# shirokumakur0/Riemannian-interior-point-trust-region-method

Measured on AMD Instinct MI355X. Metric: outer RIPTRM iterations/sec, batched NonnegPCA n=4000, 1/2/4/8 MI355X, higher is better.
Workload: dtype f64

## Files before the change

riemannian-interior-point-trust-region-method_amd/csrc/riptrm_device.h:

```cpp
#pragma once
#include <stdint.h>
#include "../../include/riptrm.h"

namespace riptrm {

constexpr int TS = 128;
constexpr int SP_WAVES = 8;
constexpr int SP_THREADS = SP_WAVES * 64;
constexpr int GV_THREADS = 256;
constexpr int GV_RW = 4;
constexpr int GV_RB = (GV_THREADS / 64) * GV_RW;
constexpr int ST_THREADS = 512;
constexpr int ST_WAVES = ST_THREADS / 64;

enum Vec : int {
  V_X = 0, V_Y, V_ETA, V_HETA,
  V_SX, V_X0, V_Y0, V_SX0, V_XPREV, V_R, V_IN0, V_IN1, V_OUT0, V_OUT1, V_YNEW, V_C,
  V_XI, V_YI, V_SXI,
  NVEC
};

enum St : int {
  ST_PHASE = 0, ST_MODE, ST_OUTER_IT, ST_INNER_IT, ST_MU_IDX, ST_MU, ST_DELTA, ST_DELTA0,
  ST_DELTA_STEP, ST_T_START, ST_T_INNER, ST_TOLL, ST_TOLC,
  ST_XX, ST_XSX, ST_YX, ST_COEF, ST_FCUR,
  ST_EPE, ST_EPD, ST_DPD, ST_ZR, ST_NORMR0, ST_MODEL, ST_J, ST_TCG_STOP,
  ST_NORMDX, ST_XDX, ST_MINX, ST_MINY, ST_COMPL, ST_XFEAS, ST_YFEAS,
  ST_HASMIN, ST_MINEIG, ST_MINEIG_OK,
  ST_HOT_END,
  ST_TCG_TOTAL = 40, ST_INNER_TOTAL, ST_PASSES, ST_LOG_COUNT, ST_LOG_OVERFLOW, ST_STOP_CODE,
  ST_STOP_RUNTIME, ST_RESIDUAL,
  ST_I_HAS, ST_I_NUM, ST_I_STATUS, ST_I_TR, ST_I_DXTYPE, ST_I_NORMDX, ST_I_MINX, ST_I_MINY,
  ST_I_COMPL, ST_I_HASRATIO, ST_I_RATIO, ST_I_RU, ST_I_DC, ST_I_HASMIN, ST_I_MINEIG,
  ST_ERROR, ST_LOG_BASE, ST_RHS,
  ST_N_USED
};
constexpr int ST_N = 72;
constexpr int ST_HOT = ST_HOT_END;
static_assert(ST_HOT_END <= 40, "hot scalar slots overflow into cold ones");
static_assert(ST_N_USED <= ST_N, "state slots overflow");

enum Phase : int {
  PH_IDLE = 0, PH_START, PH_AFTER_SX0, PH_TCG, PH_TRIAL, PH_PAUSED, PH_DONE,
  PH_TCGO_START, PH_TCGO_SX, PH_ERROR,
  PH_TRS, PH_TRS_END,
  PH_TRS_HOST, PH_MINEIG_HOST, PH_MINEIG_END
};

enum Mode : int { MODE_SOLVE = 0, MODE_TCG_ONLY = 1 };

struct Layout {
  int32_t n, batch, cap, layout, nt;
  int32_t reps;
  int64_t ld;
  int64_t off_vec, off_state, off_stats, off_log, off_pbuf, off_lists, off_req, off_cnt;
  int64_t off_rvec, off_rstate, off_rstats, off_rreq, off_pbuf2, off_sync, sync_bytes, off_tgrid, tgrid_bytes;
  int64_t total;
};

inline int64_t round_up(int64_t a, int64_t m) { return (a + m - 1) / m * m; }

__host__ __device__ inline int64_t log_slot(int64_t k, int64_t cap) {
  if (k < cap) return k;
  const int64_t h = cap / 2, t = cap - h;
  return h + (k - h) % t;
}
inline int64_t ld_of(int32_t n) { return round_up(n > 0 ? n : 1, TS); }
inline int64_t rows_of(int32_t n) { return round_up(n > 0 ? n : 1, 32); }
inline int32_t nt_of(int32_t n) { return (int32_t)(ld_of(n) / TS); }
inline int64_t ntiles_of(int32_t n) { const int64_t t = nt_of(n); return t * (t + 1) / 2; }
constexpr int SB = 2;
constexpr int SW = SB * TS;
inline int32_t nst_of(int32_t n) { return (nt_of(n) + SB - 1) / SB; }
inline int64_t nsup_of(int32_t n) { const int64_t t = nst_of(n); return t * (t + 1) / 2; }
inline int64_t pgrid_of(int32_t n) {
  const int64_t a = (int64_t)nt_of(n) * nt_of(n) * TS, b = (int64_t)nst_of(n) * nst_of(n) * SW;
  return a > b ? a : b;
}
#ifndef RIPTRM_MM_KZ
#define RIPTRM_MM_KZ 4
#endif
constexpr int MM_KZ = RIPTRM_MM_KZ;

inline int32_t edge_w_of(int32_t n) {
  return (int32_t)round_up((int64_t)(n > 0 ? n : 1) - (int64_t)(nt_of(n) - 1) * TS, 32);
}
__host__ __device__ inline int64_t sym_off(int I, int J, int nt, int wl) {
  const int64_t F = (int64_t)TS * TS;
  return F * ((int64_t)I * (nt - 1) - (int64_t)I * (I - 1) / 2) + (int64_t)I * TS * wl + (int64_t)(J - I) * F;
}

inline int64_t s_elems_of(int32_t n, int32_t layout) {
  if (layout == RIPTRM_LAYOUT_SYMTILE) {
    const int nt = nt_of(n), wl = edge_w_of(n);
    return sym_off(nt - 1, nt - 1, nt, wl) + (int64_t)wl * wl;
  }
  return rows_of(n) * ld_of(n);
}

constexpr int PERSIST_MAX_WG = 256;
constexpr int PERSIST_MAX_N = 2048;
inline int32_t persist_reps_of(int32_t n, int32_t batch, int32_t layout) {
  if (layout != RIPTRM_LAYOUT_SYMTILE || n > PERSIST_MAX_N) return 0;
  const int64_t t = ntiles_of(n);
  return (int64_t)batch * t <= PERSIST_MAX_WG ? (int32_t)t : 0;
}

inline Layout make_layout(int32_t n, int32_t batch, int32_t cap, int32_t layout) {
  Layout L;
  L.n = n; L.batch = batch; L.cap = cap; L.ld = ld_of(n); L.layout = layout; L.nt = nt_of(n);
  int64_t o = 0;
  L.off_vec = o;   o += (int64_t)NVEC * batch * L.ld * 8;               o = round_up(o, 256);
  L.off_state = o; o += (int64_t)batch * ST_N * 8;                       o = round_up(o, 256);
  L.off_stats = o; o += (int64_t)batch * RIPTRM_STAT_NFIELDS * 8;        o = round_up(o, 256);
  L.off_log = o;   o += (int64_t)batch * cap * RIPTRM_LOG_NFIELDS * 8;   o = round_up(o, 256);
  L.off_pbuf = o;
  if (layout == RIPTRM_LAYOUT_SYMTILE) o += (int64_t)2 * batch * pgrid_of(n) * 8;
  if (layout == RIPTRM_LAYOUT_SHARED) o += (int64_t)MM_KZ * 2 * batch * L.ld * 8;
  o = round_up(o, 256);
  L.off_lists = o; o += (int64_t)4 * batch * 4;                          o = round_up(o, 256);
  L.off_req = o;   o += (int64_t)batch * 4;                              o = round_up(o, 256);
  L.off_cnt = o;   o += 64;
  L.reps = persist_reps_of(n, batch, layout);
  const int64_t bs = L.reps > 0 ? (int64_t)batch * (L.reps - 1) : 0;
  L.off_rvec = o;   o += (int64_t)NVEC * bs * L.ld * 8;                  o = round_up(o, 256);
  L.off_rstate = o; o += bs * ST_N * 8;                                  o = round_up(o, 256);
  L.off_rstats = o; o += bs * RIPTRM_STAT_NFIELDS * 8;                   o = round_up(o, 256);
  L.off_rreq = o;   o += bs * 4;                                         o = round_up(o, 256);
  L.off_pbuf2 = o;  if (L.reps > 0) o += (int64_t)2 * batch * pgrid_of(n) * 8;  o = round_up(o, 256);
  L.off_sync = o;
  L.sync_bytes = L.reps > 0 ? round_up((int64_t)batch * 4, 16) + (int64_t)2 * batch * 8 + 16 : 0;
  o += L.sync_bytes;                                                     o = round_up(o, 256);
  L.off_tgrid = o;
  L.tgrid_bytes = L.reps > 0 ? (int64_t)2 * batch * nt_of(n) * nt_of(n) * TS * 16 : 0;
  o += L.tgrid_bytes;                                                    o = round_up(o, 256);
  L.total = o;
  return L;
}

struct DevParams {
  const double* S;
  int64_t inst_stride;
  int64_t ld;
  int32_t n, batch, cap;
  int32_t nrb;
  int32_t layout;
  int32_t nt;
  int32_t ntiles;
  int32_t wl;
  int32_t nst, nsup;
  int32_t smode;
  int32_t sup_dyn;
  double* pbuf;
  int32_t pbatch;
  double* vec;
  double* st;
  double* stats;
  double* log;
  int32_t* lists;
  int32_t* req;
  int32_t* cnt;
  const double* mu_tab;
  const double* tolL_tab;
  const double* tolC_tab;
  int32_t tab_len;
  int32_t outer_target;
  double clock_hz;
  int32_t trs_hbm;
  riptrm_options opt;
};

}
```

riemannian-interior-point-trust-region-method_amd/csrc/riptrm_kernels.hip:

```cpp
#include <hip/hip_runtime.h>
#include <math.h>
#include <string>
#include <vector>
#include <cstring>
#include <cstdio>
#include <type_traits>
#include "riptrm_device.h"
#include "riptrm_ctx.h"
#include "riptrm_wave.h"
#include "riptrm_trs.h"

namespace riptrm {

#pragma clang fp contract(off)

typedef double dbl2 __attribute__((ext_vector_type(2)));

__device__ __forceinline__ double* vp(const DevParams& P, int k, int b) {
  return P.vec + ((int64_t)k * P.batch + b) * P.ld;
}

__device__ __forceinline__ int32_t le_make(int b, int nrhs) { return b * 2 + (nrhs - 1); }
__device__ __forceinline__ int le_b(int32_t e) { return e >> 1; }
__device__ __forceinline__ int le_nrhs(int32_t e) { return (e & 1) + 1; }
// ... 173 lines not shown
  const int lane = (int)__lane_id();
#pragma unroll
  for (int k = 0; k < 4; ++k) {
    swap32(a[k], a[k + 4]);
    a[k] = a[k] + a[k + 4];
  }
#pragma unroll
  for (int k = 0; k < 2; ++k) {
    swap16(a[k], a[k + 2]);
    a[k] = a[k] + a[k + 2];
  }
  const double r0 = a[0], r1 = a[1];
  const bool b3 = (lane & 8) != 0;
  const double snd = b3 ? r0 : r1, kp = b3 ? r1 : r0;
  double v = kp + xor_lane(snd, 8);
  v += xor_lane(v, 4);
  v += xor_lane(v, 2);
  v += xor_lane(v, 1);
  return v;
}

template <int NR>
__device__ __forceinline__ void spass_tile(const DevParams& P, int b, int t) {
  int I, J;
  tile_ij(t, P.nt, I, J);
  const int lane = (int)__lane_id();
  const int w = __builtin_amdgcn_readfirstlane(threadIdx.x >> 6);
  const int nt = P.nt, wl = P.wl;
  const int rowsT = (I == nt - 1) ? wl : TS;
  const int colsT = (J == nt - 1) ? wl : TS;
  const bool cl = 2 * lane < colsT;
  const double* __restrict__ T = P.S + (int64_t)b * P.inst_stride + sym_off(I, J, nt, wl);
  const double* __restrict__ v0 = vp(P, V_IN0, b);
  const double* __restrict__ v1 = vp(P, V_IN1, b);
  const dbl2 vj0 = *(const dbl2*)(v0 + J * TS + 2 * lane);
  dbl2 vj1 = dbl2{0.0, 0.0};
  if (NR == 2) vj1 = *(const dbl2*)(v1 + J * TS + 2 * lane);
  const int64_t nn = (int64_t)P.nt * P.nt * TS;
  double* __restrict__ pb0 = P.pbuf + (int64_t)b * nn;
  double* __restrict__ pb1 = P.pbuf + ((int64_t)P.pbatch + b) * nn;
  double c0x = 0.0, c0y = 0.0, c1x = 0.0, c1y = 0.0;
  const int rrow = 4 * ((lane >> 5) & 1) + 2 * ((lane >> 4) & 1) + ((lane >> 3) & 1);
  constexpr int ROWS = TS / SP_WAVES;
#pragma unroll 1
  for (int rb = 0; rb < ROWS / 8; ++rb) {
    const int r0 = w * ROWS + rb * 8;
    if (r0 >= rowsT) break;
    dbl2 sv[8];
#pragma unroll
    for (int k = 0; k < 8; ++k)
      sv[k] = cl ? __builtin_nontemporal_load((const dbl2*)(T + (r0 + k) * colsT + 2 * lane)) : dbl2{0.0, 0.0};
    double a[8];
#pragma unroll
    for (int k = 0; k < 8; ++k) {
      const double vi0 = v0[I * TS + r0 + k];
      a[k] = __builtin_fma(sv[k].y, vj0.y, sv[k].x * vj0.x);
      c0x = __builtin_fma(sv[k].x, vi0, c0x);
      c0y = __builtin_fma(sv[k].y, vi0, c0y);
    }
    const double s0 = reduce_scatter8(a);
    if ((lane & 7) == 0) pb0[((int64_t)I * P.nt + J) * TS + r0 + rrow] = s0;
    if (NR == 2) {
#pragma unroll
      for (int k = 0; k < 8; ++k) {
        const double vi1 = v1[I * TS + r0 + k];
        a[k] = __builtin_fma(sv[k].y, vj1.y, sv[k].x * vj1.x);
        c1x = __builtin_fma(sv[k].x, vi1, c1x);
        c1y = __builtin_fma(sv[k].y, vi1, c1y);
      }
      const double s1 = reduce_scatter8(a);
      if ((lane & 7) == 0) pb1[((int64_t)I * P.nt + J) * TS + r0 + rrow] = s1;
    }
  }
  if (I != J) {
    __shared__ double cs[2][SP_WAVES][TS];
    cs[0][w][2 * lane] = c0x;
    cs[0][w][2 * lane + 1] = c0y;
    if (NR == 2) {
      cs[1][w][2 * lane] = c1x;
      cs[1][w][2 * lane + 1] = c1y;
    }
    __syncthreads();
    if (threadIdx.x < TS) {
      const int c = threadIdx.x;
      double s0 = cs[0][0][c];
#pragma unroll
      for (int q = 1; q < SP_WAVES; ++q) s0 += cs[0][q][c];
      pb0[((int64_t)J * P.nt + I) * TS + c] = s0;
      if (NR == 2) {
        double s1 = cs[1][0][c];
#pragma unroll
        for (int q = 1; q < SP_WAVES; ++q) s1 += cs[1][q][c];
        pb1[((int64_t)J * P.nt + I) * TS + c] = s1;
      }
    }
  }
}

__global__ void __launch_bounds__(SP_THREADS, 4) k_spass_sym(DevParams P, int list_in, int zero_cnt) {
  if (zero_cnt >= 0 && blockIdx.x == 0 && threadIdx.x == 0) P.cnt[zero_cnt] = 0;
  const int slot = blockIdx.x / P.ntiles;
  const int nact = P.cnt[list_in];
  const int32_t e = P.lists[list_in * P.batch + slot];
  if (slot >= nact) return;
  const int b = le_b(e);
  const int t = blockIdx.x - slot * P.ntiles;
  if (le_nrhs(e) == 2) spass_tile<2>(P, b, t);
  else spass_tile<1>(P, b, t);
}

constexpr int SUP_OCAP = 15360;
constexpr int SUP_MAXU = SUP_OCAP / (2 * SW);

typedef double (*sup_red_t)[SP_WAVES][SW];

template <int NR>
__device__ __forceinline__ void sup_unit(const DevParams& P, int b, int Pq, int Qq, sup_red_t red, double* out, int rsel) {
  const int lane = (int)__lane_id();
  const int w = __builtin_amdgcn_readfirstlane(threadIdx.x >> 6);
  const int nt = P.nt, wl = P.wl;
  constexpr int ROWS = TS / SP_WAVES;
  const double* __restrict__ Sb = P.S + (int64_t)b * P.inst_stride;
  const double* __restrict__ v0 = vp(P, V_IN0, b);
  const double* __restrict__ v1 = vp(P, V_IN1, b);
  const int rrow = 4 * ((lane >> 5) & 1) + 2 * ((lane >> 4) & 1) + ((lane >> 3) & 1);
  double racc[NR][SB][2];
#pragma unroll
  for (int k = 0; k < NR; ++k)
#pragma unroll
    for (int i = 0; i < SB; ++i) racc[k][i][0] = racc[k][i][1] = 0.0;
  if (NR == 2) __syncthreads();
  const int r0sel = NR == 2 ? 0 : rsel;
#pragma unroll
  for (int k = 0; k < NR; ++k)
    for (int jl = 0; jl < SB; ++jl) {
      red[r0sel + k][w][jl * TS + 2 * lane] = 0.0;
      red[r0sel + k][w][jl * TS + 2 * lane + 1] = 0.0;
    }
#pragma unroll
  for (int il = 0; il < SB; ++il) {
    const int I = SB * Pq + il;
    if (I >= nt) break;
    const int rowsT = (I == nt - 1) ? wl : TS;
    constexpr bool hoist = NR == 1;
    double vih[ROWS];
    if (hoist) {
#pragma unroll
      for (int k = 0; k < ROWS; ++k) vih[k] = v0[I * TS + w * ROWS + k];
    }
#pragma unroll 1
    for (int jl = 0; jl < SB; ++jl) {
      const int J = SB * Qq + jl;
      if (J >= nt || J < I) continue;
      const int colsT = (J == nt - 1) ? wl : TS;
      const bool cl = 2 * lane < colsT;
      const double* __restrict__ T = Sb + sym_off(I, J, nt, wl);
      const dbl2 vj0 = *(const dbl2*)(v0 + J * TS + 2 * lane);
      dbl2 vj1 = dbl2{0.0, 0.0};
      if (NR == 2) vj1 = *(const dbl2*)(v1 + J * TS + 2 * lane);
      double vi0[ROWS], vi1[ROWS];
#pragma unroll
      for (int k = 0; k < ROWS; ++k) {
        vi0[k] = hoist ? vih[k] : v0[I * TS + w * ROWS + k];
        vi1[k] = NR == 2 ? v1[I * TS + w * ROWS + k] : 0.0;
      }
      __builtin_amdgcn_sched_barrier(0);
      double c0x = 0.0, c0y = 0.0, c1x = 0.0, c1y = 0.0;
      dbl2 sv2[ROWS / 8][8];
#pragma unroll
      for (int rb = 0; rb < ROWS / 8; ++rb)
#pragma unroll
        for (int k = 0; k < 8; ++k) {
          const int row = w * ROWS + rb * 8 + k;
          const bool ok = cl && row < rowsT;
          const dbl2 x = __builtin_nontemporal_load((const dbl2*)(T + (row < rowsT ? row : 0) * colsT + (cl ? 2 * lane : 0)));
          sv2[rb][k] = ok ? x : dbl2{0.0, 0.0};
        }
#pragma unroll
      for (int rb = 0; rb < ROWS / 8; ++rb) {
        const int r0 = w * ROWS + rb * 8;
        if (r0 >= rowsT) break;
        const dbl2 (&sv)[8] = sv2[rb];
        double a[8];
#pragma unroll
        for (int k = 0; k < 8; ++k) {
          const double vi = vi0[rb * 8 + k];
          a[k] = __builtin_fma(sv[k].y, vj0.y, sv[k].x * vj0.x);
          c0x = __builtin_fma(sv[k].x, vi, c0x);
          c0y = __builtin_fma(sv[k].y, vi, c0y);
        }
        racc[0][il][rb] += reduce_scatter8(a);
        if (NR == 2) {
#pragma unroll
          for (int k = 0; k < 8; ++k) {
            const double vi = vi1[rb * 8 + k];
            a[k] = __builtin_fma(sv[k].y, vj1.y, sv[k].x * vj1.x);
            c1x = __builtin_fma(sv[k].x, vi, c1x);
            c1y = __builtin_fma(sv[k].y, vi, c1y);
          }
          racc[NR - 1][il][rb] += reduce_scatter8(a);
        }
      }
      if (I != J) {
        red[r0sel][w][jl * TS + 2 * lane] += c0x;
        red[r0sel][w][jl * TS + 2 * lane + 1] += c0y;
        if (NR == 2) {
          red[NR - 1][w][jl * TS + 2 * lane] += c1x;
          red[NR - 1][w][jl * TS + 2 * lane + 1] += c1y;
        }
      }
    }
  }
  if ((lane & 7) == 0) {
#pragma unroll
    for (int k = 0; k < NR; ++k)
#pragma unroll
      for (int il = 0; il < SB; ++il) {
        out[(2 * k) * SW + il * TS + w * ROWS + rrow] = racc[k][il][0];
        out[(2 * k) * SW + il * TS + w * ROWS + 8 + rrow] = racc[k][il][1];
      }
  }
  __syncthreads();
  for (int t = threadIdx.x; t < NR * SW; t += SP_THREADS) {
    const int k = t / SW, c = t - k * SW;
    double cs = red[r0sel + k][0][c];
#pragma unroll
    for (int q = 1; q < SP_WAVES; ++q) cs += red[r0sel + k][q][c];
    if (Pq == Qq) out[(2 * k) * SW + c] += cs;
    else out[(2 * k + 1) * SW + c] = cs;
  }
  if (NR == 2) __syncthreads();
}

__device__ __forceinline__ void sup_flush(const DevParams& P, const double* outb, const int (*meta)[2], int nslot,
                                          int list_in) {
  __syncthreads();
  const int64_t nn = (int64_t)P.nst * P.nst * SW;
  int off = 0;
  for (int s = 0; s < nslot; ++s) {
    const int u = meta[s][0], nr = meta[s][1];
    const int slot = u / P.nsup;
    const int b = le_b(P.lists[list_in * P.batch + slot]);
    int Pq, Qq;
    tile_ij(u - slot * P.nsup, P.nst, Pq, Qq);
    const int t = threadIdx.x, side = t / SW, c = t - side * SW;
    for (int k = 0; k < nr; ++k) {
      double* pb = P.pbuf + ((int64_t)k * P.pbatch + b) * nn;
      if (side == 0) pb[((int64_t)Pq * P.nst + Qq) * SW + c] = outb[off + (2 * k) * SW + c];
      else if (Pq != Qq) pb[((int64_t)Qq * P.nst + Pq) * SW + c] = outb[off + (2 * k + 1) * SW + c];
    }
    off += nr * 2 * SW;
  }
  __syncthreads();
}

__global__ void __launch_bounds__(SP_THREADS, 1) k_spass_sup(DevParams P, int list_in, int zero_cnt) {
  static_assert(SP_THREADS == 2 * SW, "sup_flush: one thread per element of the two sides");
  __shared__ double red[2][SP_WAVES][SW];
  __shared__ double outb[SUP_OCAP];
  __shared__ int meta[SUP_MAXU][2];
  __shared__ int tick_next;
  if (zero_cnt >= 0 && blockIdx.x == 0 && threadIdx.x == 0) P.cnt[zero_cnt] = 0;
  const int nact = P.cnt[list_in];
  const int total = nact * P.nsup;
  int used = 0, nslot = 0, rsel = 0;
  const bool dyn = P.sup_dyn != 0;
  unsigned int* tick = (unsigned int*)P.cnt + 8 + list_in;
  unsigned int* done = (unsigned int*)P.cnt + 12 + list_in;
  int u = blockIdx.x;
  if (dyn) {
    if (threadIdx.x == 0) tick_next = (int)atomicAdd(tick, 1u);
    __syncthreads();
    u = tick_next;
  }
  while (u < total) {
    unsigned int pre = 0;
    if (dyn && threadIdx.x == 0) pre = atomicAdd(tick, 1u);
    const int slot = u / P.nsup;
    const int32_t e = P.lists[list_in * P.batch + slot];
    const int b = le_b(e), nr = le_nrhs(e);
    int Pq, Qq;
    tile_ij(u - slot * P.nsup, P.nst, Pq, Qq);
    if (used + nr * 2 * SW > SUP_OCAP) {
      sup_flush(P, outb, meta, nslot, list_in);
      used = 0;
      nslot = 0;
    }
    if (nr == 2) {
      sup_unit<2>(P, b, Pq, Qq, red, outb + used, 0);
    } else {
      sup_unit<1>(P, b, Pq, Qq, red, outb + used, rsel);
      rsel ^= 1;
    }
    if (threadIdx.x == 0) {
      meta[nslot][0] = u;
      meta[nslot][1] = nr;
    }
    used += nr * 2 * SW;
    ++nslot;
    if (dyn) {
      __syncthreads();
      if (threadIdx.x == 0) tick_next = (int)pre;
      __syncthreads();
      u = tick_next;
    } else {
      u += gridDim.x;
    }
  }
  if (nslot > 0) sup_flush(P, outb, meta, nslot, list_in);
  if (dyn && threadIdx.x == 0) {
    if (atomicAdd(done, 1u) == gridDim.x - 1) {
      atomicExch(tick, 0u);
      atomicExch(done, 0u);
    }
  }
}

typedef double dbl4 __attribute__((ext_vector_type(4)));
typedef __attribute__((address_space(3))) unsigned char lds_u8;
#ifndef RIPTRM_MM_WAVES
#define RIPTRM_MM_WAVES 16
#endif
constexpr int MM_WAVES = RIPTRM_MM_WAVES;
typedef __attribute__((address_space(3))) dbl2 lds_dbl2;
#ifndef RIPTRM_MM_NST
#define RIPTRM_MM_NST 3
#endif

template <int N>
__device__ __forceinline__ void mm_wait_barrier() {
#define MM_WB_CASE(K) else if constexpr (N == K) asm volatile("s_waitcnt vmcnt(" #K ")\n\ts_barrier" ::: "memory");
  if constexpr (N == 0) asm volatile("s_waitcnt vmcnt(0)\n\ts_barrier" ::: "memory");
  MM_WB_CASE(1) MM_WB_CASE(2) MM_WB_CASE(3) MM_WB_CASE(4) MM_WB_CASE(5) MM_WB_CASE(6) MM_WB_CASE(7)
  MM_WB_CASE(8) MM_WB_CASE(9) MM_WB_CASE(10) MM_WB_CASE(11) MM_WB_CASE(12)
#undef MM_WB_CASE
  else static_assert(N < 0, "mm_wait_barrier: add the count");
}

template <int WM, int RT>
struct MmShape {
  static constexpr int NW = MM_WAVES;
  static constexpr int CT = 16 * WM;
  static constexpr int NWR = NW < RT / 16 ? NW : RT / 16;
  static constexpr int NWC = NW / NWR < WM ? NW / NWR : WM, NACT = NWR * NWC;
  static constexpr int WMW = WM / NWC;
  static constexpr int RW = RT / NWR, WN = RW / 16;
  static constexpr int VT = CT * 256;
  static constexpr int STAGE = VT + RT * 256;
  static constexpr int VW = NW < CT / 4 ? NW : CT / 4, VP = CT / 4 / VW;
  static constexpr int SW = NW < RT / 4 ? NW : RT / 4, SP = RT / 4 / SW;
  static constexpr int NST = RIPTRM_MM_NST >= 3 && 3 * STAGE + 32 * 4 <= 160 * 1024 ? 3 : 2;
  static_assert(WMW >= 1 && WN >= 1 && WM % NWC == 0 && VP * VW * 4 == CT && SP * SW * 4 == RT, "tile shape");
};

template <int WM, int RT, typename SlotOf>
__device__ __forceinline__ void mm_tile(const DevParams& P, lds_u8* smem, const int32_t* lst, int vk, int which, int nv,
                                        SlotOf slot_of, int z, int i0, int rows) {
  using Sh = MmShape<WM, RT>;
  constexpr int CT = Sh::CT, WN = Sh::WN, WMW = Sh::WMW, RW = Sh::RW, NWR = Sh::NWR;
  constexpr int VT = Sh::VT, STAGE = Sh::STAGE, VP = Sh::VP, SP = Sh::SP, NST = Sh::NST;
  constexpr int VW = Sh::VW, SW = Sh::SW, NACT = Sh::NACT;
  const int lane = threadIdx.x & 63, w = __builtin_amdgcn_readfirstlane((int)threadIdx.x >> 6);
  const int wr = w % NWR, wc = w / NWR;
  const int r = lane & 15, q = lane >> 4;
  const int64_t ld = P.ld;
  const double* vsrc[VP];
  const double* ssrc[SP];
#pragma unroll
  for (int p = 0; p < VP; ++p) {
    const int row = 4 * (VP * w + p) + q;
    vsrc[p] = vp(P, vk, le_b(lst[slot_of(min(row, nv - 1))])) + 2 * (r ^ (row & 15));
  }
#pragma unroll
  for (int p = 0; p < SP; ++p) {
    const int row = 4 * (SP * w + p) + q;
    const int i = min(i0 + row, rows - 1);
    ssrc[p] = P.S + (int64_t)i * ld + 2 * (r ^ (row & 15));
  }
  const int nch = (int)(ld / 32), per = (nch + MM_KZ - 1) / MM_KZ;
  const int lo = z * per, hi = min(nch, lo + per);
  auto issue = [&](int ch, int buf) {
    const int64_t k0 = (int64_t)ch * 32;
    lds_u8* vb = smem + buf * STAGE;
#pragma unroll
    for (int p = 0; p < VP; ++p)
      if (VW == Sh::NW || w < VW)
        __builtin_amdgcn_global_load_lds((const void*)(vsrc[p] + k0), vb + 4 * (VP * w + p) * 256, 16, 0, 0);
#pragma unroll
    for (int p = 0; p < SP; ++p)
      if (SW == Sh::NW || w < SW)
        __builtin_amdgcn_global_load_lds((const void*)(ssrc[p] + k0), vb + VT + 4 * (SP * w + p) * 256, 16, 0, 0);
  };
  dbl4 acc[WMW][WN];
#pragma unroll
  for (int a = 0; a < WMW; ++a)
#pragma unroll
    for (int c = 0; c < WN; ++c) acc[a][c] = dbl4{0.0, 0.0, 0.0, 0.0};
  const bool live = w < NACT && i0 + RW * wr < P.n && 16 * WMW * wc < nv;
  if (lo < hi) issue(lo, 0);
  if (NST == 3 && lo + 1 < hi) issue(lo + 1, 1);
  int s = 0;
  for (int ch = lo; ch < hi; ++ch) {
    if (NST == 3 && ch + 1 < hi) {
      if (w < VW && w < SW) mm_wait_barrier<VP + SP>();
      else if (w < VW) mm_wait_barrier<VP>();
      else if (w < SW) mm_wait_barrier<SP>();
      else mm_wait_barrier<0>();
    } else {
      mm_wait_barrier<0>();
    }
    if (ch + NST - 1 < hi) issue(ch + NST - 1, s == 0 ? NST - 1 : s - 1);
    const int sc = s;
    s = s + 1 == NST ? 0 : s + 1;
    if (!live) continue;
    const lds_u8* vb = smem + sc * STAGE + 16 * WMW * wc * 256;
    const lds_u8* sb = smem + sc * STAGE + VT + RW * wr * 256;
    dbl2 fa[2][WMW], fb[2][WN];
    auto frag = [&](int jj, int u) {
      const int off = ((4 * q + jj) ^ r) * 16;
#pragma unroll
      for (int a = 0; a < WMW; ++a) fa[u][a] = *(const lds_dbl2*)(vb + (16 * a + r) * 256 + off);
#pragma unroll
      for (int c = 0; c < WN; ++c) fb[u][c] = *(const lds_dbl2*)(sb + (16 * c + r) * 256 + off);
    };
    frag(0, 0);
#pragma unroll
    for (int jj = 0; jj < 4; ++jj) {
      const int u = jj & 1;
      if (jj < 3) frag(jj + 1, u ^ 1);
#pragma unroll
      for (int mm = 0; mm < 2; ++mm)
#pragma unroll
        for (int a = 0; a < WMW; ++a)
#pragma unroll
          for (int c = 0; c < WN; ++c)
            acc[a][c] = __builtin_amdgcn_mfma_f64_16x16x4f64(mm ? fa[u][a].y : fa[u][a].x, mm ? fb[u][c].y : fb[u][c].x,
                                                             acc[a][c], 0, 0, 0);
    }
  }
  (void)CT;
  if (!live) return;
  double* slab = P.pbuf + ((int64_t)z * 2 + which) * P.batch * ld;
#pragma unroll
  for (int a = 0; a < WMW; ++a)
#pragma unroll
    for (int g = 0; g < 4; ++g) {
      const int v = 16 * (WMW * wc + a) + q + 4 * g;
      if (v >= nv) continue;
      double* o = slab + (int64_t)le_b(lst[slot_of(v)]) * ld;
#pragma unroll
      for (int c = 0; c < WN; ++c) {
        const int i = i0 + RW * wr + 16 * c + r;
        if (i < P.n) o[i] = acc[a][c][g];
      }
    }
}

template <int WM0, int RT>
constexpr int mm_shm() { return MmShape<WM0, RT>::NST * MmShape<WM0, RT>::STAGE + 32 * 4; }
// ... 2202 lines not shown
                     c->L.reps - 1);
  HIPCHK(c, hipGetLastError());
  return RIPTRM_OK;
}

static void reset_groups(riptrm_ctx* c) {
  c->parity[0] = c->parity[1] = 0;
  c->active_bound[0] = c->active_bound[1] = 0;
}

static int kick(riptrm_ctx* c);
static int run_steps(riptrm_ctx* c, int steps, int* n_active);

extern "C++" template <int K>
static hipError_t persist_launch(riptrm_ctx* c, unsigned grid, DevParams p, RepBlock rq, PersistSync sy, int steps) {
  const size_t shm = (size_t)TS * TS * sizeof(double);
  if (c->persist_req == 2) {
    hipLaunchKernelGGL(k_persist<K>, dim3(grid), dim3(ST_THREADS), shm, c->stream, p, rq, sy, steps);
    return hipGetLastError();
  }
  if (c->persist_req == 3 && !c->persist_launched) return hipErrorCooperativeLaunchTooLarge;
  void* args[] = {&p, &rq, &sy, &steps};
  return hipLaunchCooperativeKernel((const void*)k_persist<K>, dim3(grid), dim3(ST_THREADS), args, (unsigned)shm,
                                    c->stream);
}

static int persist_run(riptrm_ctx* c, int steps, int* n_active) {
  const PersistSync sy = persist_sync(c);
  HIPCHK(c, hipMemsetAsync(c->ws + c->L.off_sync, 0, (size_t)(c->L.off_tgrid - c->L.off_sync + c->L.tgrid_bytes),
                           c->stream));
  if (steps > 0) {
    int i0 = -1, i1 = -1;
    hipEvent_t e0 = nullptr, e1 = nullptr;
    if (c->prof && (e0 = prof_event(c, &i0)) && (e1 = prof_event(c, &i1))) HIPCHK(c, hipEventRecord(e0, c->stream));
    const unsigned grid = (unsigned)(c->P.batch * c->L.reps);
    const DevParams Q = persist_params(c);
    const RepBlock rq{Q.vec, Q.st, Q.stats, Q.req, Q.batch};
    static_assert(PERSIST_MAX_N <= 4 * ST_THREADS, "k_persist<4> covers every persistent shape");
    const hipError_t le = c->P.n <= 2 * ST_THREADS ? persist_launch<2>(c, grid, params_for(c, 0), rq, sy, steps)
                                                    : persist_launch<4>(c, grid, params_for(c, 0), rq, sy, steps);
    if (le != hipSuccess) {
      (void)hipGetLastError();
      if (c->persist_launched)
        return fail(c, RIPTRM_E_HIP, std::string("persistent lock-step launch refused mid-solve: ") + hipGetErrorString(le));
      c->persist_on = false;
      c->persist_fallbacks++;
      c->ev_used -= (e0 ? 1 : 0) + (e1 ? 1 : 0);
      reset_groups(c);
      HIPCHK(c, hipMemsetAsync(c->P.cnt, 0, 4 * sizeof(int32_t), c->stream));
      if (int rc = kick(c)) return rc;
      return run_steps(c, steps, n_active);
    }
    c->persist_launched = true;
    if (c->prof && e1) {
      HIPCHK(c, hipEventRecord(e1, c->stream));
      c->ev_state.push_back({i0, i1});
    }
  }
  hipLaunchKernelGGL(k_persist_count, dim3(1), dim3(256), 0, c->stream, c->P, c->parity[0]);
  HIPCHK(c, hipGetLastError());
  int32_t h = 0;
  uint32_t flag = 0;
  HIPCHK(c, hipMemcpyAsync(&h, c->P.cnt + c->parity[0], sizeof(int32_t), hipMemcpyDeviceToHost, c->stream));
  HIPCHK(c, hipMemcpyAsync(&flag, sy.flag, sizeof(uint32_t), hipMemcpyDeviceToHost, c->stream));
  HIPCHK(c, hipStreamSynchronize(c->stream));
  if (c->prof) prof_collect(c);
  c->active_bound[0] = h;
  if (n_active) *n_active = h;
  if (flag) return fail(c, RIPTRM_E_HIP, "persistent lock-step: a workgroup waited > 2 s at an in-launch barrier "
                                        "(instance stopped with STAT_ERROR = 2)");
  return RIPTRM_OK;
}

static int calibrate_spass(riptrm_ctx* c) {
  c->sup_auto = 1;
  c->spass_cal_ms[0] = c->spass_cal_ms[1] = 0.0f;
  const int count = c->gsize[0];
  if (c->P.layout != RIPTRM_LAYOUT_SYMTILE || c->sup_req != 3 || (int64_t)count * c->P.nsup < (int64_t)4 * c->ncu)
    return RIPTRM_OK;
  hipLaunchKernelGGL(k_list_range, dim3((unsigned)((count + 255) / 256)), dim3(256), 0, c->stream, c->P, c->gbase[0], count);
  HIPCHK(c, hipGetLastError());
  hipEvent_t ev[4];
  for (auto& e : ev) HIPCHK(c, hipEventCreate(&e));
  float ms[2] = {0.0f, 0.0f};
  int rc = RIPTRM_OK;
  const bool prof = c->prof;
  c->prof = false;
  for (int kind = 0; kind < 2 && rc == RIPTRM_OK; ++kind) {
    rc = launch_gemv(c, c->stream, 0, -1, count, kind);
    if (rc == RIPTRM_OK) rc = hipEventRecord(ev[2 * kind], c->stream) == hipSuccess ? RIPTRM_OK : RIPTRM_E_HIP;
    for (int r = 0; r < 3 && rc == RIPTRM_OK; ++r) rc = launch_gemv(c, c->stream, 0, -1, count, kind);
    if (rc == RIPTRM_OK) rc = hipEventRecord(ev[2 * kind + 1], c->stream) == hipSuccess ? RIPTRM_OK : RIPTRM_E_HIP;
  }
  if (rc == RIPTRM_OK && hipEventSynchronize(ev[3]) == hipSuccess && hipEventElapsedTime(&ms[0], ev[0], ev[1]) == hipSuccess &&
      hipEventElapsedTime(&ms[1], ev[2], ev[3]) == hipSuccess)
    c->sup_auto = ms[1] <= ms[0] ? 1 : 0;
  c->spass_cal_ms[0] = ms[0] / 3.0f;
  c->spass_cal_ms[1] = ms[1] / 3.0f;
  c->prof = prof;
  for (auto& e : ev) (void)hipEventDestroy(e);
  if (rc) return rc;
  HIPCHK(c, hipMemsetAsync(c->P.cnt, 0, 4 * sizeof(int32_t), c->stream));
  return RIPTRM_OK;
}

int riptrm_nonnegpca_bind(riptrm_ctx* ctx, const double* S, int32_t n, int32_t batch, int32_t layout,
                          int64_t inst_stride, void* workspace, int64_t workspace_bytes, int32_t cap) {
  if (!ctx) return RIPTRM_E_ARG;
  if (!S || !workspace || n < 2 || batch <= 0 || cap < 0 || !layout_ok(layout))
    return fail(ctx, RIPTRM_E_ARG, "bind: bad argument (need n >= 2, batch >= 1, a known layout)");
  if (layout == RIPTRM_LAYOUT_SHARED) {
    if (inst_stride != 0) return fail(ctx, RIPTRM_E_ARG, "bind: the shared layout needs inst_stride = 0");
  } else if (inst_stride < s_elems_of(n, layout) || (inst_stride % 2) != 0) {
    return fail(ctx, RIPTRM_E_ARG, "bind: instance stride smaller than riptrm_nonnegpca_s_elems (or odd)");
  }
  if (((uintptr_t)S % 16) != 0 || ((uintptr_t)workspace % 256) != 0)
    return fail(ctx, RIPTRM_E_ARG, "bind: S must be 16-byte and workspace 256-byte aligned");
  const Layout L = make_layout(n, batch, cap, layout);
  if (workspace_bytes < L.total) return fail(ctx, RIPTRM_E_ARG, "bind: workspace too small");
  HIPCHK(ctx, hipSetDevice(ctx->device));
  HIPCHK(ctx, hipMemsetAsync(workspace, 0, (size_t)L.total, ctx->stream));
  ctx->L = L;
  ctx->S = S;
  ctx->inst_stride = inst_stride;
  ctx->ws = (char*)workspace;
  DevParams& P = ctx->P;
  std::memset(&P, 0, sizeof(P));
  P.S = S;
  P.inst_stride = inst_stride;
  P.ld = L.ld;
  P.n = n;
  P.batch = batch;
  P.cap = cap;
  P.nrb = (int)(rows_of(n) / GV_RB);
  P.layout = layout;
  P.nt = L.nt;
  P.ntiles = (int)ntiles_of(n);
  P.wl = edge_w_of(n);
  P.nst = nst_of(n);
  P.nsup = (int32_t)nsup_of(n);
  P.smode = 0;
  P.pbuf = (double*)(ctx->ws + L.off_pbuf);
  P.vec = (double*)(ctx->ws + L.off_vec);
  P.st = (double*)(ctx->ws + L.off_state);
  P.stats = (double*)(ctx->ws + L.off_stats);
  P.log = (double*)(ctx->ws + L.off_log);
  P.lists = (int32_t*)(ctx->ws + L.off_lists);
  P.req = (int32_t*)(ctx->ws + L.off_req);
  P.cnt = (int32_t*)(ctx->ws + L.off_cnt);
  P.pbatch = batch;
  {
    const char* ev = getenv("RIPTRM_SUP_DYNAMIC");
    P.sup_dyn = ev ? (atoi(ev) != 0) : 0;
  }
  P.clock_hz = ctx->clock_hz;
  P.outer_target = INT32_MAX;
  ctx->persist_ok = ctx->persist_req != 0 && L.reps > 0 && (int64_t)batch * L.reps <= ctx->ncu;
  ctx->persist_on = false;
  ctx->persist_fallbacks = 0;
  if (ctx->persist_ok) {
    HIPCHK(ctx, hipFuncSetAttribute((const void*)k_persist<2>, hipFuncAttributeMaxDynamicSharedMemorySize,
                                    (int)(TS * TS * sizeof(double))));
    HIPCHK(ctx, hipFuncSetAttribute((const void*)k_persist<4>, hipFuncAttributeMaxDynamicSharedMemorySize,
                                    (int)(TS * TS * sizeof(double))));
    int nb = 0, coop = 0;
    const void* kp = n <= 2 * ST_THREADS ? (const void*)k_persist<2> : (const void*)k_persist<4>;
    HIPCHK(ctx, hipOccupancyMaxActiveBlocksPerMultiprocessor(&nb, kp, ST_THREADS, (size_t)TS * TS * sizeof(double)));
    HIPCHK(ctx, hipDeviceGetAttribute(&coop, hipDeviceAttributeCooperativeLaunch, ctx->device));
    ctx->persist_ok = nb >= 1 && (int64_t)batch * L.reps <= (int64_t)nb * ctx->ncu && (coop || ctx->persist_req == 2);
  }
  if (layout == RIPTRM_LAYOUT_SHARED) {
    HIPCHK(ctx, hipFuncSetAttribute((const void*)k_spass_mm<8, 128>, hipFuncAttributeMaxDynamicSharedMemorySize,
                                    mm_shm<8, 128>()));
    HIPCHK(ctx, hipFuncSetAttribute((const void*)k_spass_mm<8, 64>, hipFuncAttributeMaxDynamicSharedMemorySize,
                                    mm_shm<8, 64>()));
    HIPCHK(ctx, hipFuncSetAttribute((const void*)k_spass_mm<2, 128>, hipFuncAttributeMaxDynamicSharedMemorySize,
                                    mm_shm<2, 128>()));
    HIPCHK(ctx, hipFuncSetAttribute((const void*)k_spass_mm<2, 64>, hipFuncAttributeMaxDynamicSharedMemorySize,
                                    mm_shm<2, 64>()));
  }
  ctx->ngroups = (layout != RIPTRM_LAYOUT_SHARED && batch >= 8 &&
                  (double)batch * s_elems_of(n, layout) * 8.0 >= 1.2e9) ? 2 : 1;
  if (ctx->groups_req > 0) ctx->ngroups = (ctx->groups_req >= 2 && batch >= 2) ? 2 : 1;
  ctx->gbase[0] = 0;
  ctx->gsize[0] = ctx->ngroups == 2 ? (batch + 1) / 2 : batch;
  ctx->gbase[1] = ctx->gsize[0];
  ctx->gsize[1] = batch - ctx->gsize[0];
  ctx->bound = true;
  ctx->solving = false;
  ctx->pver++;
  return calibrate_spass(ctx);
}

constexpr int SUP_MIN_UNITS = 64;
static int spass_mode(const riptrm_ctx* c, int bound) {
  if (c->P.layout != RIPTRM_LAYOUT_SYMTILE || c->sup_req == 0) return 0;
  if (c->sup_req == 2) return 1;
  if (c->sup_req == 1) return c->P.nsup >= SUP_MIN_UNITS ? 1 : 0;
  const bool wide = (int64_t)bound * c->P.nsup >= (int64_t)c->ncu;
  return (wide && c->sup_auto) ? 1 : 0;
}

static DevParams params_for(const riptrm_ctx* c, int smode) {
  DevParams P = c->P;
  P.smode = smode;
  return P;
}

static int launch_gemv(riptrm_ctx* c, hipStream_t st, int list_in, int zero_cnt, int bound, int smode) {
  if (bound <= 0) return RIPTRM_OK;
  const bool sym = c->P.layout == RIPTRM_LAYOUT_SYMTILE;
  const int64_t blocks = (int64_t)bound * (sym ? c->P.ntiles : c->P.nrb);
  int i0 = -1, i1 = -1;
  hipEvent_t e0 = nullptr, e1 = nullptr;
  if (c->prof && (e0 = prof_event(c, &i0)) && (e1 = prof_event(c, &i1))) HIPCHK(c, hipEventRecord(e0, st));
  if (c->P.layout == RIPTRM_LAYOUT_SHARED) {
    const int rows = rows_of(c->P.n);
    const bool rt128 = (int64_t)((rows + 127) / 128) * MM_KZ >= c->ncu;
    const int nrb = rt128 ? (rows + 127) / 128 : (rows + 63) / 64;
    const int t0 = bound > 32 ? (bound + 127) / 128 : (bound + 31) / 32;
    const dim3 grid((unsigned)(nrb * t0 * MM_KZ));
    if (bound > 32) {
      if (rt128)
        hipLaunchKernelGGL((k_spass_mm<8, 128>), grid, dim3(64 * MM_WAVES), (mm_shm<8, 128>()), st, c->P, list_in, zero_cnt, bound);
      else
        hipLaunchKernelGGL((k_spass_mm<8, 64>), grid, dim3(64 * MM_WAVES), (mm_shm<8, 64>()), st, c->P, list_in, zero_cnt, bound);
    } else {
      if (rt128)
        hipLaunchKernelGGL((k_spass_mm<2, 128>), grid, dim3(64 * MM_WAVES), (mm_shm<2, 128>()), st, c->P, list_in, zero_cnt, bound);
      else
        hipLaunchKernelGGL((k_spass_mm<2, 64>), grid, dim3(64 * MM_WAVES), (mm_shm<2, 64>()), st, c->P, list_in, zero_cnt, bound);
    }
  } else if (sym && smode) {
    const int64_t units = (int64_t)bound * c->P.nsup;
    const unsigned grid = (unsigned)(units < c->ncu ? units : c->ncu);
    hipLaunchKernelGGL(k_spass_sup, dim3(grid), dim3(SP_THREADS), 0, st, params_for(c, 1), list_in, zero_cnt);
  } else if (sym)
    hipLaunchKernelGGL(k_spass_sym, dim3((unsigned)blocks), dim3(SP_THREADS), 0, st, c->P, list_in, zero_cnt);
  else
    hipLaunchKernelGGL(k_gemv, dim3((unsigned)blocks), dim3(GV_THREADS), 0, st, c->P, list_in, zero_cnt);
  HIPCHK(c, hipGetLastError());
  if (c->prof && e1) {
    HIPCHK(c, hipEventRecord(e1, st));
    c->ev_gemv.push_back({i0, i1});
  }
  return RIPTRM_OK;
}

static size_t state_lds_bytes(const DevParams& P) {
  if (P.opt.trs_solver != RIPTRM_TRS_SOLVER_EXACT_REPMAT || P.n - 1 > riptrm_trs::DIM_MAX) return 0;
  return ((size_t)riptrm_trs::work_doubles(P.n - 1) + 2 * (riptrm_trs::DIM_MAX + 1) + 2 * ST_WAVES) * sizeof(double);
}

static int launch_state(riptrm_ctx* c, hipStream_t st, int full, int list_in, int list_out, int bound,
                        int full_base, int smode) {
  const int blocks = bound;
  if (blocks <= 0) return RIPTRM_OK;
  int i0 = -1, i1 = -1;
  hipEvent_t e0 = nullptr, e1 = nullptr;
  if (c->prof && (e0 = prof_event(c, &i0)) && (e1 = prof_event(c, &i1))) HIPCHK(c, hipEventRecord(e0, st));
  if (c->P.opt.trs_solver == RIPTRM_TRS_SOLVER_EXACT_REPMAT)
    hipLaunchKernelGGL(k_state<true>, dim3((unsigned)blocks), dim3(ST_THREADS), state_lds_bytes(c->P), st,
                       params_for(c, smode), full,
                       list_in, list_out, full_base, bound);
  else
    hipLaunchKernelGGL(k_state<false>, dim3((unsigned)blocks), dim3(ST_THREADS), 0, st, params_for(c, smode), full,
                       list_in, list_out,
                       full_base, bound);
  HIPCHK(c, hipGetLastError());
  if (c->prof && e1) {
    HIPCHK(c, hipEventRecord(e1, st));
    c->ev_state.push_back({i0, i1});
  }
  return RIPTRM_OK;
}

static int fork_streams(riptrm_ctx* c) {
  c->gstream[0] = c->stream;
  c->gstream[1] = c->own_stream;
  if (c->ngroups < 2) return RIPTRM_OK;
  HIPCHK(c, hipEventRecord(c->ev_fork, c->stream));
  HIPCHK(c, hipStreamWaitEvent(c->own_stream, c->ev_fork, 0));
  return RIPTRM_OK;
}

static int join_streams(riptrm_ctx* c) {
  if (c->ngroups < 2) return RIPTRM_OK;
  HIPCHK(c, hipEventRecord(c->ev_join, c->own_stream));
  HIPCHK(c, hipStreamWaitEvent(c->stream, c->ev_join, 0));
  return RIPTRM_OK;
}

int riptrm_nonnegpca_hvp(riptrm_ctx* ctx, const double* x, const double* y, double mu, const double* v, double* out, int64_t ldv) {
  if (!ctx) return RIPTRM_E_ARG;
  if (!ctx->bound) return fail(ctx, RIPTRM_E_STATE, "hvp: bind first");
  if (!x || !y || !v || !out || ldv < ctx->P.n) return fail(ctx, RIPTRM_E_ARG, "hvp: bad argument");
  HIPCHK(ctx, hipSetDevice(ctx->device));
  const int B = ctx->P.batch;
  hipLaunchKernelGGL(k_hvp_prep, dim3(B), dim3(256), 0, ctx->stream, ctx->P, x, y, v, ldv);
  HIPCHK(ctx, hipGetLastError());
  const int sm = spass_mode(ctx, B);
  int rc = launch_gemv(ctx, ctx->stream, 0, -1, B, sm);
  if (rc) return rc;
  hipLaunchKernelGGL(k_hvp_epi, dim3(B), dim3(ST_THREADS), 0, ctx->stream, params_for(ctx, sm), mu, out, ldv);
  HIPCHK(ctx, hipGetLastError());
  ctx->solving = false;
// ... 335 lines not shown
```

Before: 3097.

## Skip lower triangle loads in diagonal super tiles and add cost-balanced partition

Diagonal tiles in the symmetric matvec now load only the upper triangle per lane by offsetting the column start, masking the lower entries and adding the diagonal contribution separately. This lets diagonal tiles feed the transposed reduction as well, with no special case. A new opt-in mode (RIPTRM_SUP_BALANCED) builds a per-super-tile cost prefix sum in shared memory and gives each block a contiguous, roughly equal-cost range of units instead of a round-robin stride. The triangle change always runs and is meant to cut memory traffic on diagonal tiles. The balanced split is off by default and adds a prefix scan plus binary search per block.

```diff
diff --git a/riemannian-interior-point-trust-region-method_amd/csrc/riptrm_device.h b/riemannian-interior-point-trust-region-method_amd/csrc/riptrm_device.h
--- a/riemannian-interior-point-trust-region-method_amd/csrc/riptrm_device.h
+++ b/riemannian-interior-point-trust-region-method_amd/csrc/riptrm_device.h
@@ -151,6 +151,7 @@
   int32_t nst, nsup;
   int32_t smode;
   int32_t sup_dyn;
+  int32_t sup_bal;
   double* pbuf;
   int32_t pbatch;
   double* vec;
diff --git a/riemannian-interior-point-trust-region-method_amd/csrc/riptrm_kernels.hip b/riemannian-interior-point-trust-region-method_amd/csrc/riptrm_kernels.hip
--- a/riemannian-interior-point-trust-region-method_amd/csrc/riptrm_kernels.hip
+++ b/riemannian-interior-point-trust-region-method_amd/csrc/riptrm_kernels.hip
@@ -349,8 +349,11 @@
     for (int jl = 0; jl < SB; ++jl) {
       const int J = SB * Qq + jl;
       if (J >= nt || J < I) continue;
+      const bool dg = I == J;
       const int colsT = (J == nt - 1) ? wl : TS;
       const bool cl = 2 * lane < colsT;
+      const bool wst = w * ROWS < rowsT;
+      const int co = max(cl ? 2 * lane : 0, dg && wst ? w * ROWS : 0);
       const double* __restrict__ T = Sb + sym_off(I, J, nt, wl);
       const dbl2 vj0 = *(const dbl2*)(v0 + J * TS + 2 * lane);
       dbl2 vj1 = dbl2{0.0, 0.0};
@@ -361,6 +364,15 @@
         vi0[k] = hoist ? vih[k] : v0[I * TS + w * ROWS + k];
         vi1[k] = NR == 2 ? v1[I * TS + w * ROWS + k] : 0.0;
       }
+      double d0 = 0.0, d1 = 0.0;
+      if (dg) {
+        const bool has = cl && wst && (lane >> 3) == w;
+        const int dl = has ? 2 * lane : wst ? w * ROWS : 0;
+        const dbl2 e0 = __builtin_nontemporal_load((const dbl2*)(T + dl * colsT + dl));
+        const dbl2 e1 = __builtin_nontemporal_load((const dbl2*)(T + (dl + 1) * colsT + dl));
+        d0 = has ? e0.x : 0.0;
+        d1 = has ? e1.y : 0.0;
+      }
       __builtin_amdgcn_sched_barrier(0);
       double c0x = 0.0, c0y = 0.0, c1x = 0.0, c1y = 0.0;
       dbl2 sv2[ROWS / 8][8];
@@ -370,9 +382,19 @@
         for (int k = 0; k < 8; ++k) {
           const int row = w * ROWS + rb * 8 + k;
           const bool ok = cl && row < rowsT;
-          const dbl2 x = __builtin_nontemporal_load((const dbl2*)(T + (row < rowsT ? row : 0) * colsT + (cl ? 2 * lane : 0)));
+          const dbl2 x = __builtin_nontemporal_load((const dbl2*)(T + (row < rowsT ? row : 0) * colsT + co));
           sv2[rb][k] = ok ? x : dbl2{0.0, 0.0};
         }
+      if (dg) {
+        const int kd = 2 * (lane - 8 * w);
+#pragma unroll
+        for (int rb = 0; rb < ROWS / 8; ++rb)
+#pragma unroll
+          for (int k = 0; k < 8; ++k) {
+            sv2[rb][k].x = kd > rb * 8 + k ? sv2[rb][k].x : 0.0;
+            sv2[rb][k].y = kd >= rb * 8 + k ? sv2[rb][k].y : 0.0;
+          }
+      }
 #pragma unroll
       for (int rb = 0; rb < ROWS / 8; ++rb) {
         const int r0 = w * ROWS + rb * 8;
@@ -398,13 +420,19 @@
           racc[NR - 1][il][rb] += reduce_scatter8(a);
         }
       }
-      if (I != J) {
-        red[r0sel][w][jl * TS + 2 * lane] += c0x;
-        red[r0sel][w][jl * TS + 2 * lane + 1] += c0y;
+      if (dg) {
+        c0x = __builtin_fma(d0, vj0.x, c0x);
+        c0y = __builtin_fma(d1, vj0.y, c0y);
         if (NR == 2) {
-          red[NR - 1][w][jl * TS + 2 * lane] += c1x;
-          red[NR - 1][w][jl * TS + 2 * lane + 1] += c1y;
+          c1x = __builtin_fma(d0, vj1.x, c1x);
+          c1y = __builtin_fma(d1, vj1.y, c1y);
         }
+      }
+      red[r0sel][w][jl * TS + 2 * lane] += c0x;
+      red[r0sel][w][jl * TS + 2 * lane + 1] += c0y;
+      if (NR == 2) {
+        red[NR - 1][w][jl * TS + 2 * lane] += c1x;
+        red[NR - 1][w][jl * TS + 2 * lane + 1] += c1y;
       }
     }
   }
@@ -450,6 +478,33 @@
   }
   __syncthreads();
 }
+
+__device__ __forceinline__ int sup_unit_lines(int Pq, int Qq, int nt, int wl) {
+  int lines = 0;
+  for (int il = 0; il < SB; ++il)
+    for (int jl = 0; jl < SB; ++jl) {
+      const int I = SB * Pq + il, J = SB * Qq + jl;
+      if (I >= nt || J >= nt || J < I) continue;
+      const int rows = (I == nt - 1) ? wl : TS, m = ((J == nt - 1) ? wl : TS) / 16;
+      lines += rows * m - (I == J ? 8 * m * (m - 1) : 0);
+    }
+  return lines;
+}
+
+__device__ __forceinline__ int sup_bal_first(const int* pre, int nsup, int64_t x) {
+  const int C = pre[nsup];
+  const int slot = (int)(x / C);
+  const int rem = (int)(x - (int64_t)slot * C);
+  int lo = 0, hi = nsup;
+  while (lo < hi) {
+    const int mid = (lo + hi) >> 1;
+    if (pre[mid] >= rem) hi = mid;
+    else lo = mid + 1;
+  }
+  return slot * nsup + lo;
+}
+
+constexpr int SUP_BAL_MAX = 512;
 
 __global__ void __launch_bounds__(SP_THREADS, 1) k_spass_sup(DevParams P, int list_in, int zero_cnt) {
   static_assert(SP_THREADS == 2 * SW, "sup_flush: one thread per element of the two sides");
@@ -470,7 +525,34 @@
     __syncthreads();
     u = tick_next;
   }
-  while (u < total) {
+  __shared__ int bal_pre[SUP_BAL_MAX + 1];
+  __shared__ int bal_wtot[SP_WAVES];
+  int uend = total, ustep = gridDim.x;
+  if (!dyn && P.sup_bal != 0 && P.nsup <= SUP_BAL_MAX && total > (int)gridDim.x) {
+    static_assert(SUP_BAL_MAX <= SP_THREADS, "one thread per table entry");
+    const int t = threadIdx.x, lane = t & 63, w = t >> 6;
+    int c = 0;
+    if (t < P.nsup) {
+      int Pq, Qq;
+      tile_ij(t, P.nst, Pq, Qq);
+      c = sup_unit_lines(Pq, Qq, P.nt, P.wl);
+    }
+    for (int d = 1; d < 64; d <<= 1) {
+      const int o = __shfl_up(c, d);
+      if (lane >= d) c += o;
+    }
+    if (lane == 63) bal_wtot[w] = c;
+    __syncthreads();
+    for (int q = 0; q < w; ++q) c += bal_wtot[q];
+    if (t < P.nsup) bal_pre[t + 1] = c;
+    if (t == 0) bal_pre[0] = 0;
+    __syncthreads();
+    const int64_t T = (int64_t)nact * bal_pre[P.nsup], G = gridDim.x, g = blockIdx.x;
+    u = sup_bal_first(bal_pre, P.nsup, (g * T + G - 1) / G);
+    uend = sup_bal_first(bal_pre, P.nsup, ((g + 1) * T + G - 1) / G);
+    ustep = 1;
+  }
+  while (u < uend) {
     unsigned int pre = 0;
     if (dyn && threadIdx.x == 0) pre = atomicAdd(tick, 1u);
     const int slot = u / P.nsup;
@@ -501,7 +583,7 @@
       __syncthreads();
       u = tick_next;
     } else {
-      u += gridDim.x;
+      u += ustep;
     }
   }
   if (nslot > 0) sup_flush(P, outb, meta, nslot, list_in);
@@ -3010,6 +3092,8 @@
   {
     const char* ev = getenv("RIPTRM_SUP_DYNAMIC");
     P.sup_dyn = ev ? (atoi(ev) != 0) : 0;
+    ev = getenv("RIPTRM_SUP_BALANCED");
+    P.sup_bal = ev ? (atoi(ev) != 0) : 0;
   }
   P.clock_hz = ctx->clock_hz;
   P.outer_target = INT32_MAX;
```

After: 3092. No clear change (-0.2%).
